# uwoseis/zephyr

Hardware: AMD Instinct MI355X
Metric: wavefields/sec (freq x source solves/s) on 1024^2 grid (higher is better)
Workload: dtype f64

## Files before the change

__graft_entry__.py:

```python
import os
import subprocess
import sys

ROOT = os.path.dirname(os.path.abspath(__file__))
CSRC = os.path.join(ROOT, 'zephyr_amd', 'csrc')
LIB = os.path.join(ROOT, 'zephyr_amd', 'libhelm.so')
SOURCES = ['assemble.hip', 'stencil.hip', 'vector.hip', 'mg.hip', 'helm3d.hip', 'mg3d.hip', 'mg3_keep.hip', 'mg3_coarse.hip', 'mg3_depth.hip', 'nd_plan.hip', 'nd_gemm.hip', 'nd_gj.hip', 'nd_leaf.hip', 'nd_factor.hip',
           'nd_passes.hip', 'nd_resid.hip', 'regrid.hip', 'runtime.hip', 'krylov.hip', 'solve_direct.hip', 'capi.hip', 'survey.hip', 'survey_frechet.hip', 'survey_hessian.hip', 'survey_newton.hip', 'survey_joint.hip',
           'survey_visco.hip', 'survey_eurus.hip']
HEADERS = ['helm_internal.hpp', 'mz_row.hpp', 'eu_row.hpp', 'solve_internal.hpp', 'mg3_internal.hpp', 'direct.hpp', 'nd_internal.hpp', 'nd_gemm_body.hpp', 'nd_gj32w.hpp', 'survey_internal.hpp']
HIPCC = os.environ.get('HIPCC', '/opt/rocm/bin/hipcc')
FLAGS = ['--offload-arch=gfx950', '-O3', '-std=c++17', '-fPIC', '-ffp-contract=fast-honor-pragmas', '-Wno-unused-value', '-Wno-unused-result']


def _stale(target, deps):
    if not os.path.exists(target):
        return True
    t = os.path.getmtime(target)
    return any(os.path.getmtime(d) > t for d in deps)


def _write_build_info(objs, ran):
    import time
    lines = ['libhelm build record (written by __graft_entry__.build())', 'hipcc: %s' % HIPCC, 'flags: %s' % ' '.join(FLAGS), '']
    lines += ['commands run by the last build that compiled something:'] + (['  ' + c.replace(ROOT + os.sep, '') for c in ran] or ['  (none: everything was up to date)'])
    lines += ['', 'artefacts:']
    for pth in objs + [LIB]:
        if os.path.exists(pth):
            st = os.stat(pth)
            lines.append('  %-40s %10d bytes  %s' % (os.path.relpath(pth, ROOT), st.st_size, time.strftime('%Y-%m-%d %H:%M:%S', time.gmtime(st.st_mtime))))
    try:
        open(os.path.join(CSRC, 'BUILD_INFO.txt'), 'w').write('\n'.join(lines) + '\n')
    except OSError:
        pass


def build(force=False):
    srcs = [os.path.join(CSRC, s) for s in SOURCES]
    hdrs = [os.path.join(CSRC, h) for h in HEADERS] + [os.path.join(ROOT, 'include', 'helm.h')]
    objs, ran, todo = [], [], []
    for s in srcs:
        o = s[:-4] + '.o'
        if force or _stale(o, [s] + hdrs):
# ... 62 lines not shown
```

include/helm.h:

```cpp
#ifndef HELM_H
#define HELM_H

#include <stddef.h>

#ifdef __cplusplus
extern "C" {
#endif

typedef struct helm_op helm_op;

enum { HELM_MINIZEPHYR = 0, HELM_EURUS = 1, HELM_3D = 2  };

enum {
    HELM_BICGSTAB = 0,
    HELM_CGNR = 1,
    HELM_AUTO = 2,
    HELM_MG = 3,
    HELM_DIRECT = 4
};

enum {
    HELM_OK = 0,
    HELM_ERR_ARG = -1,
    HELM_ERR_DEVICE = -2,
// ... 207 lines not shown
    int    nd_sparse_rhs;
    int    nd_stable;
    double nd_stable_thr;
    double nd_stable_safety;
    int    nd_fused_leaf;
    int    nd_fused_leaf_min;
    int    nd_gjstep;
    int    nd_gjstep_min;
    int    nd_overlap;
    int    nd_xcd_map;
    int    nd_plans;
    int    nd_direct_out;
    int    nd_many;
    int    nd_leaf_idle;
    int    auto_direct;
    int    auto_mg3;
    int    prof_ext;
    int    ws_slots;
    int    pf_prio;
    int    mg3_keep;
    int    mg3_keep_levels;
    int    mg3_galerkin;
    int    mg3_depth_model;
    int    mg3_bt_f32;
    int    mg3_otf;
    int    mg3_f32;
    double mg3_omega;
    int    mg3_coarse;
    int    mg3_nd_leaf;
    int    mg3_bt_twist;
    double mg3_beta;
    double sync_spin_ms;
    int    sync_sleep_us;
    int    nd_fused_sep;
    int    nd_fused_sep_min;
} helm_tuning;
int helm_get_tuning(helm_tuning *out);
int helm_set_tuning(const helm_tuning *t);

int helm_direct_plan(int nz, int nx, int leaf, int *out, int cap);
int helm_direct_plan_front(int nz, int nx, int leaf, int node, long long *cells, int cap);
int helm_debug_zgemm(int device, int M, int N, int K, const double *alpha, const double *A, const double *B,
                     const double *beta, double *C, int batch);
int helm_debug_inverse(int device, int n, double *A, int batch);
int helm_debug_zgemm_bench(int device, int M, int N, int K, int batch, int variant, int reps, double *ms_out);
#define HELM_ZG_TABLE 1
#define HELM_ZG_MASKS 2
#define HELM_ZG_TM64  4
int helm_debug_zgemm_choice(int M, int N, int K, int batch, int nf_div, int force_tile, int force_slab, int have_handle, int mode, int report[5]);
typedef struct helm_zgemm_ex {
    int device, M, N, K, batch;
    int lda, ldb, ldc;
    long long sa, sb, sc;
    double alpha[2], beta[2];
    const double *A; long long a_len;
    double *B; long long b_len;
    double *C; long long c_len;
    int force_tile, force_slab;
    int xcd_map;
    int ntc;
    int zr0, zr1, zc0, zc1, sk0, sk1;
    int tm64, c_is_b;
    const int *tabB, *tabCi, *tabCo; long long tab_len;
    int tab_stride, offB, offCi, offCo;
    int ldx; long long arena_rows;
    const double *Bx, *Bx2, *Cix;
    double *Cox, *Cox2;
    int k2, cj_out; double oscale[2];
    int *act;
    int report[5];
} helm_zgemm_ex;
int helm_debug_zgemm_ex(helm_zgemm_ex *p);
#define HELM_NM_RESID         0
#define HELM_NM_PREP          1
#define HELM_NM_PACK          2
#define HELM_NM_SCATTER_ADD   3
#define HELM_NM_RECOVER_X     4
#define HELM_NM_TRANSPOSE_OUT 5
#define HELM_NM_TRANSPOSE     6
typedef struct helm_nm_stage {
    int device, stage, nz, nx;
    long long N;
    int ncol, nblk_cap;
    const double *planes; long long planes_len;
    const double *Xin; long long xin_len; int ldin;
    double *Q; long long q_len; int ldq;
    const int *qmap;
    int store, qnorm, xin_is_u, conj;
    double *Rout; long long rout_len;
    double *Uout; long long uout_len; int ldu;
    double oscale[2];
    const unsigned char *qmask;
    long long rhs_ld, row_off;
    double *rr, *qq;
    int report[5];
} helm_nm_stage;
int helm_debug_nm_stage(helm_nm_stage *p);
int helm_debug_inverse_bench(int device, int n, const double *A, int reps, int recurse_n, double *ms_out);

int helm_mg3_axis(int n, int npml, double h, double cpml, double om_re, double om_im, int level, double *x, int *lay, double *lap,
                  int *pc, double *pw, int *n_next, int *rf, double *rw);

int helm_regrid_axis(int n_in, double h_in, int n_out, double h_out, int *start, double *taps, int cap);
typedef struct helm_regrid helm_regrid;
helm_regrid *helm_regrid_create(int device, int nz_a, int nx_a, double dz_a, double dx_a, int nz_b, int nx_b, double dz_b, double dx_b,
                                double zorig, double xorig);
void helm_regrid_destroy(helm_regrid *plan);
int helm_regrid_axis_t(int n_in, double h_in, int n_out, double h_out, int *start, double *taps, int cap);
helm_regrid *helm_regrid_create_t(int device, int nz_a, int nx_a, double dz_a, double dx_a, int nz_b, int nx_b, double dz_b, double dx_b,
                                  double zorig, double xorig);
int helm_regrid_apply_device(helm_regrid *plan, helm_op *op, int k, const void *dIn, long long in_fstride, long long in_estride, void *dOut,
                             long long out_fstride, long long out_estride, double gain_re, double gain_im, double beta, const void *dMul);
int helm_regrid_apply(helm_regrid *plan, int k, const double *in, long long in_fstride, long long in_estride, double *out, long long out_fstride,
                      long long out_estride, double gain_re, double gain_im, double beta, const double *mul);

#ifdef __cplusplus
}
#endif
#endif
```

zephyr_amd/_lib.py:

```python
import ctypes
import os
import numpy as np

_HERE = os.path.dirname(os.path.abspath(__file__))
LIB_PATH = os.path.join(_HERE, 'libhelm.so')

HELM_MINIZEPHYR, HELM_EURUS, HELM_3D = 0, 1, 2
HELM_BICGSTAB, HELM_CGNR, HELM_AUTO, HELM_MG, HELM_DIRECT = 0, 1, 2, 3, 4
HELM_RHS_NODE_MAJOR, HELM_OUT_NODE_MAJOR, HELM_NODE_MAJOR = 1, 2, 3
METHODS = {'bicgstab': HELM_BICGSTAB, 'cgnr': HELM_CGNR, 'auto': HELM_AUTO, 'mg': HELM_MG, 'direct': HELM_DIRECT}

ERRORS = {-1: 'HELM_ERR_ARG', -2: 'HELM_ERR_DEVICE', -3: 'HELM_ERR_STATE', -4: 'HELM_ERR_UNSUPPORTED', -5: 'HELM_ERR_PML'}


class HelmError(RuntimeError):
    def __init__(self, code, text):
        self.code = code
        RuntimeError.__init__(self, '%s: %s' % (ERRORS.get(code, code), text))


class SolveOpts(ctypes.Structure):
    _fields_ = [('method', ctypes.c_int), ('rtol', ctypes.c_double), ('maxit', ctypes.c_int),
                ('check_every', ctypes.c_int), ('batch', ctypes.c_int), ('flags', ctypes.c_int)]


class SolveInfo(ctypes.Structure):
    _fields_ = [('iterations', ctypes.c_int), ('status', ctypes.c_int), ('restarts', ctypes.c_int),
                ('method', ctypes.c_int), ('relres', ctypes.c_double)]


class Timing(ctypes.Structure):
    _fields_ = [('solve_ms', ctypes.c_double), ('apply_ms', ctypes.c_double),
                ('apply_launches', ctypes.c_longlong), ('apply_bytes', ctypes.c_double),
                ('factor_ms', ctypes.c_double), ('gemm_ms', ctypes.c_double),
                ('gemm_launches', ctypes.c_longlong), ('gemm_flops', ctypes.c_double),
                ('gemm_big_ms', ctypes.c_double), ('gemm_big_launches', ctypes.c_longlong), ('gemm_big_flops', ctypes.c_double),
                ('gemm_bytes', ctypes.c_double), ('gemm_sol_ms', ctypes.c_double)]


class Tuning(ctypes.Structure):
    _fields_ = [('nd_leaf', ctypes.c_int), ('nd_ws_gb', ctypes.c_double), ('nd_sparse_rhs', ctypes.c_int), ('nd_stable', ctypes.c_int),
                ('nd_stable_thr', ctypes.c_double), ('nd_stable_safety', ctypes.c_double), ('nd_fused_leaf', ctypes.c_int),
                ('nd_fused_leaf_min', ctypes.c_int), ('nd_gjstep', ctypes.c_int), ('nd_gjstep_min', ctypes.c_int), ('nd_overlap', ctypes.c_int),
                ('nd_xcd_map', ctypes.c_int), ('nd_plans', ctypes.c_int), ('nd_direct_out', ctypes.c_int), ('nd_many', ctypes.c_int), ('nd_leaf_idle', ctypes.c_int), ('auto_direct', ctypes.c_int),
                ('auto_mg3', ctypes.c_int), ('prof_ext', ctypes.c_int), ('ws_slots', ctypes.c_int), ('pf_prio', ctypes.c_int),
                ('mg3_keep', ctypes.c_int), ('mg3_keep_levels', ctypes.c_int), ('mg3_galerkin', ctypes.c_int), ('mg3_depth_model', ctypes.c_int),
                ('mg3_bt_f32', ctypes.c_int), ('mg3_otf', ctypes.c_int), ('mg3_f32', ctypes.c_int), ('mg3_omega', ctypes.c_double),
                ('mg3_coarse', ctypes.c_int), ('mg3_nd_leaf', ctypes.c_int), ('mg3_bt_twist', ctypes.c_int), ('mg3_beta', ctypes.c_double), ('sync_spin_ms', ctypes.c_double), ('sync_sleep_us', ctypes.c_int),
                ('nd_fused_sep', ctypes.c_int), ('nd_fused_sep_min', ctypes.c_int)]


class RuntimeStats(ctypes.Structure):
    _fields_ = [('dev_allocs', ctypes.c_longlong), ('dev_alloc_bytes', ctypes.c_double), ('dev_alloc_ms', ctypes.c_double),
                ('host_allocs', ctypes.c_longlong), ('host_alloc_bytes', ctypes.c_double), ('host_alloc_ms', ctypes.c_double),
                ('events_created', ctypes.c_longlong), ('streams_created', ctypes.c_longlong),
                ('first_launches', ctypes.c_longlong), ('first_launch_ms', ctypes.c_double),
                ('kernels_registered', ctypes.c_longlong), ('kernels_resolved', ctypes.c_longlong), ('warm_ms', ctypes.c_double),
                ('dev_frees', ctypes.c_longlong), ('dev_free_ms', ctypes.c_double),
                ('sync_calls', ctypes.c_longlong), ('sync_ms', ctypes.c_double), ('slow_syncs', ctypes.c_longlong), ('worst_sync_ms', ctypes.c_double)]


class ZgemmEx(ctypes.Structure):
    _fields_ = [('device', ctypes.c_int), ('M', ctypes.c_int), ('N', ctypes.c_int), ('K', ctypes.c_int), ('batch', ctypes.c_int),
                ('lda', ctypes.c_int), ('ldb', ctypes.c_int), ('ldc', ctypes.c_int),
                ('sa', ctypes.c_longlong), ('sb', ctypes.c_longlong), ('sc', ctypes.c_longlong),
                ('alpha', ctypes.c_double * 2), ('beta', ctypes.c_double * 2),
                ('A', ctypes.c_void_p), ('a_len', ctypes.c_longlong), ('B', ctypes.c_void_p), ('b_len', ctypes.c_longlong),
                ('C', ctypes.c_void_p), ('c_len', ctypes.c_longlong),
                ('force_tile', ctypes.c_int), ('force_slab', ctypes.c_int), ('xcd_map', ctypes.c_int), ('ntc', ctypes.c_int),
                ('zr0', ctypes.c_int), ('zr1', ctypes.c_int), ('zc0', ctypes.c_int), ('zc1', ctypes.c_int), ('sk0', ctypes.c_int), ('sk1', ctypes.c_int),
                ('tm64', ctypes.c_int), ('c_is_b', ctypes.c_int),
                ('tabB', ctypes.c_void_p), ('tabCi', ctypes.c_void_p), ('tabCo', ctypes.c_void_p), ('tab_len', ctypes.c_longlong),
                ('tab_stride', ctypes.c_int), ('offB', ctypes.c_int), ('offCi', ctypes.c_int), ('offCo', ctypes.c_int),
                ('ldx', ctypes.c_int), ('arena_rows', ctypes.c_longlong),
                ('Bx', ctypes.c_void_p), ('Bx2', ctypes.c_void_p), ('Cix', ctypes.c_void_p), ('Cox', ctypes.c_void_p), ('Cox2', ctypes.c_void_p),
                ('k2', ctypes.c_int), ('cj_out', ctypes.c_int), ('oscale', ctypes.c_double * 2),
                ('act', ctypes.c_void_p), ('report', ctypes.c_int * 5)]


_c_dp = ctypes.POINTER(ctypes.c_double)
_SIGNATURES = {
    'helm_device_count': (ctypes.c_int, []),
# ... 139 lines not shown
    'helm_imaging_accumulate_c64_device': (ctypes.c_int, [ctypes.c_void_p, ctypes.c_void_p, ctypes.c_void_p, ctypes.c_void_p, ctypes.c_int,
                                                          ctypes.c_void_p, ctypes.c_void_p]),
    'helm_sample_rows_c64_device': (ctypes.c_int, [ctypes.c_void_p, ctypes.c_void_p, ctypes.c_void_p, ctypes.c_int, ctypes.c_longlong, ctypes.c_void_p,
                                                   ctypes.c_void_p, ctypes.c_void_p, ctypes.c_int, ctypes.c_longlong, ctypes.c_double, ctypes.c_double,
                                                   ctypes.c_double, ctypes.c_double, ctypes.c_void_p]),
    'helm_direct_plan': (ctypes.c_int, [ctypes.c_int, ctypes.c_int, ctypes.c_int, ctypes.c_void_p, ctypes.c_int]),
    'helm_direct_plan_front': (ctypes.c_int, [ctypes.c_int, ctypes.c_int, ctypes.c_int, ctypes.c_int, ctypes.c_void_p, ctypes.c_int]),
    'helm_mg3_axis': (ctypes.c_int, [ctypes.c_int, ctypes.c_int, ctypes.c_double, ctypes.c_double, ctypes.c_double, ctypes.c_double, ctypes.c_int,
                                     ctypes.c_void_p, ctypes.c_void_p, ctypes.c_void_p, ctypes.c_void_p, ctypes.c_void_p, ctypes.c_void_p, ctypes.c_void_p,
                                     ctypes.c_void_p]),
    'helm_debug_zgemm': (ctypes.c_int, [ctypes.c_int, ctypes.c_int, ctypes.c_int, ctypes.c_int, ctypes.c_void_p, ctypes.c_void_p,
                                        ctypes.c_void_p, ctypes.c_void_p, ctypes.c_void_p, ctypes.c_int]),
    'helm_debug_zgemm_choice': (ctypes.c_int, [ctypes.c_int] * 9 + [ctypes.POINTER(ctypes.c_int)]),
    'helm_debug_zgemm_ex': (ctypes.c_int, [ctypes.POINTER(ZgemmEx)]),
    'helm_debug_nm_stage': (ctypes.c_int, [ctypes.c_void_p]),
    'helm_debug_inverse': (ctypes.c_int, [ctypes.c_int, ctypes.c_int, ctypes.c_void_p, ctypes.c_int]),
    'helm_debug_zgemm_bench': (ctypes.c_int, [ctypes.c_int, ctypes.c_int, ctypes.c_int, ctypes.c_int, ctypes.c_int, ctypes.c_int, ctypes.c_int,
                                              ctypes.POINTER(ctypes.c_double)]),
    'helm_set_rhs_support': (ctypes.c_int, [ctypes.c_void_p, ctypes.c_void_p, ctypes.c_longlong, ctypes.c_int]),
    'helm_rhs_support_from_coo': (ctypes.c_int, [ctypes.c_void_p, ctypes.c_void_p, ctypes.c_void_p, ctypes.c_longlong, ctypes.c_void_p, ctypes.c_longlong, ctypes.c_int]),
    'helm_regrid_axis': (ctypes.c_int, [ctypes.c_int, ctypes.c_double, ctypes.c_int, ctypes.c_double, ctypes.c_void_p, ctypes.c_void_p, ctypes.c_int]),
    'helm_regrid_create': (ctypes.c_void_p, [ctypes.c_int, ctypes.c_int, ctypes.c_int, ctypes.c_double, ctypes.c_double, ctypes.c_int, ctypes.c_int,
                                             ctypes.c_double, ctypes.c_double, ctypes.c_double, ctypes.c_double]),
    'helm_regrid_axis_t': (ctypes.c_int, [ctypes.c_int, ctypes.c_double, ctypes.c_int, ctypes.c_double, ctypes.c_void_p, ctypes.c_void_p, ctypes.c_int]),
    'helm_regrid_create_t': (ctypes.c_void_p, [ctypes.c_int, ctypes.c_int, ctypes.c_int, ctypes.c_double, ctypes.c_double, ctypes.c_int, ctypes.c_int,
                                               ctypes.c_double, ctypes.c_double, ctypes.c_double, ctypes.c_double]),
    'helm_regrid_destroy': (None, [ctypes.c_void_p]),
    'helm_regrid_apply_device': (ctypes.c_int, [ctypes.c_void_p, ctypes.c_void_p, ctypes.c_int, ctypes.c_void_p, ctypes.c_longlong, ctypes.c_longlong,
                                                ctypes.c_void_p, ctypes.c_longlong, ctypes.c_longlong, ctypes.c_double, ctypes.c_double, ctypes.c_double,
                                                ctypes.c_void_p]),
    'helm_regrid_apply': (ctypes.c_int, [ctypes.c_void_p, ctypes.c_int, ctypes.c_void_p, ctypes.c_longlong, ctypes.c_longlong, ctypes.c_void_p,
                                         ctypes.c_longlong, ctypes.c_longlong, ctypes.c_double, ctypes.c_double, ctypes.c_double, ctypes.c_void_p]),
    'helm_debug_inverse_bench': (ctypes.c_int, [ctypes.c_int, ctypes.c_int, ctypes.c_void_p, ctypes.c_int, ctypes.c_int, ctypes.POINTER(ctypes.c_double)]),
}

_lib = None


def exported_symbols():
    return sorted(_SIGNATURES)


def load():
    global _lib
    if _lib is None:
        if os.environ.get('HELM_NO_TORCH_PRELOAD', '0') != '1':
            try:
                import torch
            except Exception:
                pass
        if not os.path.exists(LIB_PATH):
            raise ImportError('libhelm.so not found at %s: run `python -c "import __graft_entry__ as g; g.build()"` '
                              '(hipcc --offload-arch=gfx950).  There is no CPU fallback.' % LIB_PATH)
        lib = ctypes.CDLL(LIB_PATH)
        for name, (res, args) in _SIGNATURES.items():
            fn = getattr(lib, name)
            fn.restype = res
            fn.argtypes = args
        _lib = lib
    return _lib


def tuning():
    t = Tuning()
    check(load().helm_get_tuning(ctypes.byref(t)))
    return t
# ... 133 lines not shown
```

zephyr_amd/csrc/nd_factor.hip:

```cpp
#include "nd_internal.hpp"
#include <map>
#include <mutex>
#include <cstring>

namespace {

__device__ __forceinline__ long long mf_off(long long off, long long slot, int nf, int kf) { return (long long)nf * off + (long long)kf * slot; }
__device__ __forceinline__ cplx *front_entry(const NdDev &n, cplx *arenaF, cplx *fac, int r, int c, int nf = 1, int kf = 0, int fac_private = 0) {
    const int nmax = n.smax + n.mmax;
    if (r < n.smax) {
        return fac + (fac_private ? n.finv_off : mf_off(n.finv_off, (long long)n.smax * nmax, nf, kf)) + (long long)r * nmax + c;
    }
    return arenaF + mf_off(n.foff, (long long)n.mmax * nmax, nf, kf) + (long long)(r - n.smax) * nmax + c;
}

__global__ __launch_bounds__(256) void k_nd_assemble(const NdDev *nodes, int first, cplx *arenaF, cplx *fac, const cplx *planes, int nz, int nx) {
    const NdDev n = nodes[first + blockIdx.y];
    const long long N = (long long)nz * nx;
    const int tot = n.s + n.m;
    for (int a = blockIdx.x * blockDim.x + threadIdx.x; a < n.smax; a += gridDim.x * blockDim.x)
        if (a >= n.s) *front_entry(n, arenaF, fac, a, a) = cmake(1.0, 0.0);
    for (int a = blockIdx.x * blockDim.x + threadIdx.x; a < tot; a += gridDim.x * blockDim.x) {
        int z, x, ca;
        nd_cell(n, a, z, x, ca);
// ... 269 lines not shown
                for (int q = 0; q < NK; ++q) { const int k = p + 16 * q; if (k < i) cfma(acc, rb[u][q], Bt[k][cl]); }
                load_row(rb[u], i + PD, 0, i + PD);
                #pragma unroll
                for (int off = 8; off > 0; off >>= 1) { acc.x += __shfl_xor(acc.x, off); acc.y += __shfl_xor(acc.y, off); }
                if (p == 0) Bt[i][cl] = csub(Bt[i][cl], acc);
                __builtin_amdgcn_wave_barrier();
            }
        }
    }
    #pragma unroll
    for (int u = 0; u < PD; ++u) load_row(rb[u], n - 1 - u, n - 1 - u, n);
    for (int i0 = n - 1; i0 >= 0; i0 -= PD) {
        #pragma unroll
        for (int u = 0; u < PD; ++u) {
            const int i = i0 - u;
            if (i >= 0) {
                cplx acc = cmake(0.0, 0.0), d = cmake(1.0, 0.0);
                #pragma unroll
                for (int q = 0; q < NK; ++q) { const int k = p + 16 * q; if (k > i && k < n) cfma(acc, rb[u][q], Bt[k][cl]); if (k == i) d = rb[u][q]; }
                load_row(rb[u], i - PD, i - PD, n);
                #pragma unroll
                for (int off = 8; off > 0; off >>= 1) { acc.x += __shfl_xor(acc.x, off); acc.y += __shfl_xor(acc.y, off); }
                const int src = (lane & 48) | (i & 15);
                const double dx = __shfl(d.x, src), dy = __shfl(d.y, src);
                if (p == 0) Bt[i][cl] = cmul(csub(Bt[i][cl], acc), crecip(cmake(dx, dy)));
                __builtin_amdgcn_wave_barrier();
            }
        }
    }
    __syncthreads();
    for (int e = tid; e < n * 16; e += 256) { const int i = e >> 4, c = e & 15; if (j0 + c < ncols) B[(long long)i * ldb + j0 + c] = Bt[i][c]; }
}

}

void launch_lu_solve(hipStream_t st, const cplx *LU, int ld, int n, const int *piv, cplx *B, int ldb, int ncols) {
    HELM_LAUNCH(k_lu_solve, dim3((ncols + 15) / 16), dim3(256), 0, st, LU, ld, n, piv, B, ldb, ncols);
}

static void stable_free(NdFactor *f) {
    const int dev = f->pd ? f->pd->device : 0;
    for (NdStable &st : f->stable) {
        const size_t nmax = (size_t)st.smax + st.mmax;
        helm_pool_free(dev, st.lu, (size_t)st.smax * nmax * sizeof(cplx));
        helm_pool_free(dev, st.f21, (size_t)std::max(1, st.mmax) * st.smax * sizeof(cplx));
        helm_pool_free(dev, st.piv, (size_t)st.smax * sizeof(int));
        helm_pool_free(dev, st.vs, st.vs_elems * sizeof(cplx));
    }
    f->stable.clear();
}

struct FlagSlot { int *host = nullptr; hipEvent_t ev = nullptr; int device = 0; };
namespace { std::mutex g_flag_mu; std::map<int, std::vector<FlagSlot *>> g_flag_idle; }
FlagSlot *flag_slot_acquire(int device) {
    {
        std::lock_guard<std::mutex> lk(g_flag_mu);
        std::vector<FlagSlot *> &idle = g_flag_idle[device];
        if (!idle.empty()) { FlagSlot *s = idle.back(); idle.pop_back(); return s; }
    }
    FlagSlot *s = new FlagSlot(); s->device = device;
    s->host = (int *)helm_hostpool_alloc((ND_STABLE_CAP + 1) * sizeof(int));
    if (!s->host) { delete s; return nullptr; }
    if (hipEventCreateWithFlags(&s->ev, hipEventDisableTiming) != hipSuccess) { (void)hipGetLastError(); helm_hostpool_free(s->host, (ND_STABLE_CAP + 1) * sizeof(int)); delete s; return nullptr; }
    return s;
}
void flag_slot_release(FlagSlot *s) {
    if (!s) return;
    std::lock_guard<std::mutex> lk(g_flag_mu);
    g_flag_idle[s->device].push_back(s);
}
// ... 83 lines not shown
    {
        const hipError_t es = hipEventSynchronize(slot->ev);
        memcpy(h_list, slot->host, sizeof(h_list));
        f->flag_slot = nullptr; flag_slot_release(slot);
        if (es != hipSuccess) HELM_FAIL(op, HELM_ERR_DEVICE, "direct solver: waiting for the list of ill-conditioned fronts failed: %s", hipGetErrorString(es));
    }
    const int nflag = std::max(0, std::min(h_list[0], ND_STABLE_CAP));
    if (h_list[0] > ND_STABLE_CAP) {
        std::vector<double> eh(2 * (size_t)nf * g.cnt);
        HIP_TRY(op, hipStreamSynchronize(st));
        HIP_TRY(op, hipMemcpy(eh.data(), est, eh.size() * sizeof(double), hipMemcpyDeviceToHost));
        const double thr = f->flag_thr;
        std::vector<std::pair<double, int>> cand;
        for (int j = 0; j < g.cnt; ++j) {
            const double e = eh[(size_t)j * nf + kf] * eh[(size_t)nf * g.cnt + (size_t)j * nf + kf];
            if (!(e <= thr)) cand.push_back(std::make_pair(e == e ? e : HUGE_VAL, j));
        }
        auto worse = [](const std::pair<double, int> &a, const std::pair<double, int> &b) { return a.first != b.first ? a.first > b.first : a.second < b.second; };
        const int take = std::min<int>(nflag, (int)cand.size());
        std::partial_sort(cand.begin(), cand.begin() + take, cand.end(), worse);
        for (int q = 0; q < take; ++q) h_list[1 + q] = cand[q].second;
    }
    std::sort(h_list + 1, h_list + 1 + nflag);
    if (getenv("HELM_ND_DEBUG") && atoi(getenv("HELM_ND_DEBUG")) >= 2) {
        std::vector<double> h(2 * (size_t)nf * g.cnt);
        hipStreamSynchronize(st);
        hipMemcpy(h.data(), est, h.size() * sizeof(double), hipMemcpyDeviceToHost);
        double worst = 0; int wj = 0;
        for (int j = 0; j < g.cnt; ++j) { const double e = h[(size_t)j * nf + kf] * h[(size_t)nf * g.cnt + (size_t)j * nf + kf]; if (!(e <= worst)) { worst = e; wj = j; } }
        fprintf(stderr, "[helm direct] level %d s %d cnt %d (frequency %d of %d): estimate of front 0 = %.3e * %.3e; worst %.3e at %d; flagged %d\n", g.level, g.smax, g.cnt, kf, nf, h[kf], h[(size_t)nf * g.cnt + kf], worst, wj, h_list[0]);
    }
    if ((long long)g.smax * g.mmax > P.work_elems) return HELM_OK;
    const cplx one = cmake(1, 0), mone = cmake(-1, 0);
    for (int q = 0; q < nflag; ++q) {
        const int j = h_list[1 + q];
        NdStable S;
        S.node = g.first + j; S.group = gi; S.smax = g.smax; S.mmax = g.mmax;
        S.lu = (cplx *)helm_pool_alloc(op->device, (size_t)g.smax * nmax * sizeof(cplx));
        S.f21 = (cplx *)helm_pool_alloc(op->device, (size_t)std::max(1, g.mmax) * g.smax * sizeof(cplx));
        S.piv = (int *)helm_pool_alloc(op->device, (size_t)g.smax * sizeof(int));
        f->stable.push_back(S);
        if (!S.lu || !S.f21 || !S.piv) HELM_FAIL(op, HELM_ERR_DEVICE, "direct solver: allocation for an ill-conditioned front failed");
        NdDev n = P.nodes[S.node];
        const long long foff = (long long)nf * n.foff + (long long)kf * g.mmax * nmax;
        n.finv_off = 0; n.f12_off = g.smax;
        const int rb = std::max(std::min(nmax, 4), (nmax + 2047) / 2048);
        NdPlanesSet ps; for (int q2 = 0; q2 < ND_NF_MAX; ++q2) ps.p[q2] = planes;
        HELM_LAUNCH(k_nd_build_front<true>, dim3((nmax + rb - 1) / rb, 1), dim3(256), (size_t)nmax * sizeof(int2), st, f->pd->d_nodes, 0, arenaF, S.lu, ps, P.nz, P.nx, rb,
                           0, n, nf, kf);
        cplx *F21 = arenaF + foff, *F22 = arenaF + foff + g.smax;
        HIP_TRY(op, hipMemcpy2DAsync(S.f21, (size_t)g.smax * sizeof(cplx), F21, (size_t)nmax * sizeof(cplx), (size_t)g.smax * sizeof(cplx), (size_t)g.mmax, hipMemcpyDeviceToDevice, st));
        if (g.smax <= 64) HELM_LAUNCH(k_lu_factor64, dim3(1), dim3(256), 0, st, S.lu, nmax, g.smax, S.piv);
        else HELM_LAUNCH(k_lu_factor, dim3(1), dim3(256), 0, st, S.lu, nmax, g.smax, S.piv);
        HIP_TRY(op, hipMemcpy2DAsync(work, (size_t)g.mmax * sizeof(cplx), S.lu + g.smax, (size_t)nmax * sizeof(cplx), (size_t)g.mmax * sizeof(cplx), (size_t)g.smax, hipMemcpyDeviceToDevice, st));
        HELM_LAUNCH(k_lu_solve, dim3((g.mmax + 15) / 16), dim3(256), 0, st, (const cplx *)S.lu, nmax, g.smax, (const int *)S.piv, work, g.mmax, g.mmax);
        gemm(op, g.mmax, g.mmax, g.smax, mone, S.f21, g.smax, 0, work, g.mmax, 0, one, F22, nmax, 0, 1, nullptr);
        if (getenv("HELM_ND_DEBUG") && atoi(getenv("HELM_ND_DEBUG")) >= 3) {
            auto sum2d = [&](const void *src, size_t pitch, size_t wbytes, size_t rows_) {
                std::vector<unsigned char> h(wbytes * rows_);
                hipMemcpy2D(h.data(), wbytes, src, pitch, wbytes, rows_, hipMemcpyDeviceToHost);
                unsigned long long x = 1469598103934665603ull;
                for (unsigned char c : h) { x ^= c; x *= 1099511628211ull; }
                return x;
            };
            hipStreamSynchronize(st);
            fprintf(stderr, "[helm direct] treated front %d (level %d, s %d of %d, m %d of %d): lu %016llx f12w %016llx piv %016llx f21 %016llx work %016llx f22 %016llx\n", S.node, g.level, n.s, g.smax, n.m, g.mmax,
                    sum2d(S.lu, (size_t)nmax * sizeof(cplx), (size_t)g.smax * sizeof(cplx), g.smax), sum2d(S.lu + g.smax, (size_t)nmax * sizeof(cplx), (size_t)g.mmax * sizeof(cplx), g.smax),
                    sum2d(S.piv, (size_t)g.smax * sizeof(int), (size_t)g.smax * sizeof(int), 1),
                    sum2d(S.f21, (size_t)g.smax * sizeof(cplx), (size_t)g.smax * sizeof(cplx), g.mmax), sum2d(work, (size_t)g.mmax * sizeof(cplx), (size_t)g.mmax * sizeof(cplx), g.smax),
                    sum2d(F22, (size_t)nmax * sizeof(cplx), (size_t)g.mmax * sizeof(cplx), g.mmax));
        }
    }
    const int dbg = getenv("HELM_ND_DEBUG") ? atoi(getenv("HELM_ND_DEBUG")) : 0;
    if (dbg && nflag) fprintf(stderr, "[helm direct] level %d (%s, s = %d, m = %d): %d ill-conditioned front(s) re-eliminated with a pivoted LU\n", g.level, g.leaf ? "leaves" : "separators", g.smax, g.mmax, nflag);
    return check_kernels(op, "re-elimination of ill-conditioned fronts");
}

}

int factor_group_set(helm_op *op, const FacSet &S, size_t gi, cplx *arenaF, cplx *work) {
    NdFactor *f0 = S.f[0];
    const int nf = S.nf;
    const NdPlan &P = f0->pd->plan;
    const NdDev *d_nodes = f0->pd->d_nodes;
    hipStream_t st = op->stream;
    const cplx one = cmake(1, 0), mone = cmake(-1, 0), zero = cmake(0, 0);
    const NdGroup &g = P.groups[gi];
    const int nmax = g.smax + g.mmax;
// ... 203 lines not shown
```

zephyr_amd/csrc/runtime.hip:

```cpp
#include "helm_internal.hpp"
#include <chrono>
#include <atomic>
#include <unistd.h>
#include <time.h>
#include <mutex>
#include <thread>
#include <map>
#include <cstring>
#include <algorithm>

namespace {
struct KernelRec { const void *fn; const char *pretty; std::atomic<bool> launched{false}; };
struct KernelRegistry {
    std::mutex mu;
    std::vector<KernelRec *> recs;
    std::atomic<KernelRec *> fast[2048];
    std::atomic<int> n{0};
};
KernelRegistry &kreg() { static KernelRegistry *r = new KernelRegistry(); return *r; }
struct RuntimeCounters {
    std::atomic<long long> dev_frees{0}, dev_free_us{0}, sync_calls{0}, sync_us{0}, slow_syncs{0}, worst_sync_us{0};
    std::atomic<long long> dev_allocs{0}, dev_alloc_bytes{0}, dev_alloc_us{0}, host_allocs{0}, host_alloc_bytes{0}, host_alloc_us{0},
                           events{0}, streams{0}, first_launches{0}, first_launch_us{0}, resolved{0}, warm_us{0};
};
// ... 191 lines not shown
    t.nd_sparse_rhs = helm_env_int("HELM_ND_SPARSE_RHS", 1);
    t.nd_stable = helm_env_int("HELM_ND_STABLE", 1);
    t.nd_stable_thr = tune_d("HELM_ND_STABLE_THR", 0.0);
    t.nd_stable_safety = tune_d("HELM_ND_STABLE_SAFETY", 8.0);
    t.nd_fused_leaf = helm_env_int("HELM_ND_FUSEDLEAF", 1);
    t.nd_fused_leaf_min = helm_env_int("HELM_ND_FUSEDLEAF_MIN", 2048);
    t.nd_gjstep = helm_env_int("HELM_ND_GJSTEP", 1);
    t.nd_gjstep_min = helm_env_int("HELM_ND_GJSTEP_MIN", 128);
    t.nd_overlap = helm_env_int("HELM_ND_OVERLAP_NM", 1);
    t.nd_xcd_map = helm_env_int("HELM_ND_XCDMAP", 2);
    t.nd_plans = helm_env_int("HELM_ND_PLANS", 6);
    t.nd_direct_out = helm_env_int("HELM_ND_DIRECT_OUT", 1);
    t.nd_leaf_idle = helm_env_int("HELM_ND_LEAF_IDLE", 1);
    t.nd_many = helm_env_int("HELM_ND_MANY", 1);
    t.auto_direct = helm_env_int("HELM_AUTO_DIRECT", 1);
    t.auto_mg3 = helm_env_int("HELM_AUTO_MG3", 1);
    t.prof_ext = helm_env_int("HELM_PROF_EXT", 1);
    t.ws_slots = helm_env_int("HELM_WS_SLOTS", 3);
    t.pf_prio = helm_env_int("HELM_PF_PRIO", 1);
    t.mg3_keep = helm_env_int("HELM_MG3_KEEP", 1);
    t.mg3_keep_levels = helm_env_int("HELM_MG3_KEEP_LEVELS", -1);
    t.mg3_galerkin = helm_env_int("HELM_MG3_GALERKIN", 1);
    t.mg3_depth_model = helm_env_int("HELM_MG3_DEPTH_MODEL", 1);
    t.mg3_bt_f32 = helm_env_int("HELM_MG3_BT_F32", 1);
    t.mg3_otf = helm_env_int("HELM_MG3_OTF", 1);
    t.mg3_f32 = helm_env_int("HELM_MG3_F32", 1);
    t.mg3_omega = tune_d("HELM_MG3_OMEGA", 0.9);
    { const char *cs = getenv("HELM_MG3_COARSE"); t.mg3_coarse = cs && !strcmp(cs, "nd") ? 1 : (cs && !strcmp(cs, "bt") ? 2 : 0); }
    t.mg3_nd_leaf = helm_env_int("HELM_MG3_ND_LEAF", 2);
    t.mg3_bt_twist = helm_env_int("HELM_MG3_BT_TWIST", 1);
    t.mg3_beta = tune_d("HELM_MG3_BETA", 0.0);
    t.sync_spin_ms = tune_d("HELM_SYNC_SPIN_MS", 0.0);
    t.sync_sleep_us = helm_env_int("HELM_SYNC_SLEEP_US", 0);
    t.nd_fused_sep = helm_env_int("HELM_ND_FUSEDSEP", 1);
    t.nd_fused_sep_min = helm_env_int("HELM_ND_FUSEDSEP_MIN", 512);
    tuning_clamp(t);
    return t;
}
extern char **environ;
static unsigned long long env_fingerprint() {
    unsigned long long h = 1469598103934665603ull;
    for (char **e = environ; e && *e; ++e) {
        const char *s = *e;
        if (s[0] != 'H' || s[1] != 'E' || s[2] != 'L' || s[3] != 'M' || s[4] != '_') continue;
        for (; *s; ++s) { h ^= (unsigned char)*s; h *= 1099511628211ull; }
        h ^= 0xff; h *= 1099511628211ull;
    }
    return h;
}
static bool g_tune_have = false; static unsigned long long g_tune_fp = 0; static helm_tuning g_tune_cached;
void helm_tuning_refresh() {
    std::lock_guard<std::mutex> lk(g_tune_mu);
    const unsigned long long now = env_fingerprint();
    if (!g_tune_have || now != g_tune_fp) { g_tune_cached = tuning_from_env(); g_tune_fp = now; g_tune_have = true; }
}
helm_tuning helm_tuning_now() {
    std::lock_guard<std::mutex> lk(g_tune_mu);
    if (g_tune_set) return g_tune_user;
    if (!g_tune_have) { g_tune_cached = tuning_from_env(); g_tune_fp = env_fingerprint(); g_tune_have = true; }
    return g_tune_cached;
}
extern "C" int helm_get_tuning(helm_tuning *out) { if (!out) return HELM_ERR_ARG; helm_tuning_refresh(); *out = helm_tuning_now(); return HELM_OK; }
extern "C" int helm_set_tuning(const helm_tuning *t) {
    std::lock_guard<std::mutex> lk(g_tune_mu);
    if (t) { g_tune_user = *t; tuning_clamp(g_tune_user); g_tune_set = true; } else g_tune_set = false;
    return HELM_OK;
// ... 524 lines not shown
```

Before: 16350.

## Add blocked panel LU factor and blocked triangular solve kernels for ND fronts

Adds a panel-blocked single-workgroup LU factorization that keeps a 16-column panel and U block row in shared memory, with register-tiled trailing updates. It also adds a blocked forward/back substitution that keeps the right-hand side tile in LDS and prefetches the next L/U block. Both are enabled by default through a new tuning flag and are used in the nested-dissection stable-front path and in launch_lu_solve. The intent is to cut global-memory traffic and synchronisation in small dense LU work. The cost is more LDS per block and more intricate pivot bookkeeping.

```diff
diff --git a/__graft_entry__.py b/__graft_entry__.py
--- a/__graft_entry__.py
+++ b/__graft_entry__.py
@@ -8,7 +8,7 @@
 SOURCES = ['assemble.hip', 'stencil.hip', 'vector.hip', 'mg.hip', 'helm3d.hip', 'mg3d.hip', 'mg3_keep.hip', 'mg3_coarse.hip', 'mg3_depth.hip', 'nd_plan.hip', 'nd_gemm.hip', 'nd_gj.hip', 'nd_leaf.hip', 'nd_factor.hip',
            'nd_passes.hip', 'nd_resid.hip', 'regrid.hip', 'runtime.hip', 'krylov.hip', 'solve_direct.hip', 'capi.hip', 'survey.hip', 'survey_frechet.hip', 'survey_hessian.hip', 'survey_newton.hip', 'survey_joint.hip',
            'survey_visco.hip', 'survey_eurus.hip']
-HEADERS = ['helm_internal.hpp', 'mz_row.hpp', 'eu_row.hpp', 'solve_internal.hpp', 'mg3_internal.hpp', 'direct.hpp', 'nd_internal.hpp', 'nd_gemm_body.hpp', 'nd_gj32w.hpp', 'survey_internal.hpp']
+HEADERS = ['helm_internal.hpp', 'mz_row.hpp', 'eu_row.hpp', 'solve_internal.hpp', 'mg3_internal.hpp', 'direct.hpp', 'nd_internal.hpp', 'nd_gemm_body.hpp', 'nd_gj32w.hpp', 'nd_lu_onchip.hpp', 'survey_internal.hpp']
 HIPCC = os.environ.get('HIPCC', '/opt/rocm/bin/hipcc')
 FLAGS = ['--offload-arch=gfx950', '-O3', '-std=c++17', '-fPIC', '-ffp-contract=fast-honor-pragmas', '-Wno-unused-value', '-Wno-unused-result']
 
diff --git a/include/helm.h b/include/helm.h
--- a/include/helm.h
+++ b/include/helm.h
@@ -263,6 +263,7 @@
     double mg3_beta;
     double sync_spin_ms;
     int    sync_sleep_us;
+    int    nd_lu_onchip;
     int    nd_fused_sep;
     int    nd_fused_sep_min;
 } helm_tuning;
@@ -328,6 +329,8 @@
 } helm_nm_stage;
 int helm_debug_nm_stage(helm_nm_stage *p);
 int helm_debug_inverse_bench(int device, int n, const double *A, int reps, int recurse_n, double *ms_out);
+int helm_debug_lu(int device, int n, int ld, double *A, int *piv_out, double *B, int ldb, int ncols, int onchip);
+int helm_debug_lu_bench(int device, int n, int ld, int ncols, int onchip, int reps, double *ms_factor, double *ms_solve);
 
 int helm_mg3_axis(int n, int npml, double h, double cpml, double om_re, double om_im, int level, double *x, int *lay, double *lap,
                   int *pc, double *pw, int *n_next, int *rf, double *rw);
diff --git a/zephyr_amd/_lib.py b/zephyr_amd/_lib.py
--- a/zephyr_amd/_lib.py
+++ b/zephyr_amd/_lib.py
@@ -47,7 +47,7 @@
                 ('mg3_keep', ctypes.c_int), ('mg3_keep_levels', ctypes.c_int), ('mg3_galerkin', ctypes.c_int), ('mg3_depth_model', ctypes.c_int),
                 ('mg3_bt_f32', ctypes.c_int), ('mg3_otf', ctypes.c_int), ('mg3_f32', ctypes.c_int), ('mg3_omega', ctypes.c_double),
                 ('mg3_coarse', ctypes.c_int), ('mg3_nd_leaf', ctypes.c_int), ('mg3_bt_twist', ctypes.c_int), ('mg3_beta', ctypes.c_double), ('sync_spin_ms', ctypes.c_double), ('sync_sleep_us', ctypes.c_int),
-                ('nd_fused_sep', ctypes.c_int), ('nd_fused_sep_min', ctypes.c_int)]
+                ('nd_lu_onchip', ctypes.c_int), ('nd_fused_sep', ctypes.c_int), ('nd_fused_sep_min', ctypes.c_int)]
 
 
 class RuntimeStats(ctypes.Structure):
@@ -253,6 +253,9 @@
     'helm_regrid_apply': (ctypes.c_int, [ctypes.c_void_p, ctypes.c_int, ctypes.c_void_p, ctypes.c_longlong, ctypes.c_longlong, ctypes.c_void_p,
                                          ctypes.c_longlong, ctypes.c_longlong, ctypes.c_double, ctypes.c_double, ctypes.c_double, ctypes.c_void_p]),
     'helm_debug_inverse_bench': (ctypes.c_int, [ctypes.c_int, ctypes.c_int, ctypes.c_void_p, ctypes.c_int, ctypes.c_int, ctypes.POINTER(ctypes.c_double)]),
+    'helm_debug_lu': (ctypes.c_int, [ctypes.c_int, ctypes.c_int, ctypes.c_int, ctypes.c_void_p, ctypes.c_void_p, ctypes.c_void_p, ctypes.c_int, ctypes.c_int, ctypes.c_int]),
+    'helm_debug_lu_bench': (ctypes.c_int, [ctypes.c_int, ctypes.c_int, ctypes.c_int, ctypes.c_int, ctypes.c_int, ctypes.c_int, ctypes.POINTER(ctypes.c_double),
+                                           ctypes.POINTER(ctypes.c_double)]),
 }
 
 _lib = None
diff --git a/zephyr_amd/csrc/nd_factor.hip b/zephyr_amd/csrc/nd_factor.hip
--- a/zephyr_amd/csrc/nd_factor.hip
+++ b/zephyr_amd/csrc/nd_factor.hip
@@ -325,10 +325,76 @@
     for (int e = tid; e < n * 16; e += 256) { const int i = e >> 4, c = e & 15; if (j0 + c < ncols) B[(long long)i * ldb + j0 + c] = Bt[i][c]; }
 }
 
+
+#include "nd_lu_onchip.hpp"
+
+void launch_lu_factor_sel(hipStream_t st, cplx *A, int ld, int n, int *piv, int onchip) {
+    if (onchip) HELM_LAUNCH(k_lu_factor_onchip, dim3(1), dim3(256), 0, st, A, ld, n, piv);
+    else if (n <= 64) HELM_LAUNCH(k_lu_factor64, dim3(1), dim3(256), 0, st, A, ld, n, piv);
+    else HELM_LAUNCH(k_lu_factor, dim3(1), dim3(256), 0, st, A, ld, n, piv);
+}
+void launch_lu_solve_sel(hipStream_t st, const cplx *LU, int ld, int n, const int *piv, cplx *B, int ldb, int ncols, int onchip) {
+    if (onchip) HELM_LAUNCH(k_lu_solve_blocked, dim3((ncols + 15) / 16), dim3(256), 0, st, LU, ld, n, piv, B, ldb, ncols);
+    else HELM_LAUNCH(k_lu_solve, dim3((ncols + 15) / 16), dim3(256), 0, st, LU, ld, n, piv, B, ldb, ncols);
+}
+
 }
 
 void launch_lu_solve(hipStream_t st, const cplx *LU, int ld, int n, const int *piv, cplx *B, int ldb, int ncols) {
-    HELM_LAUNCH(k_lu_solve, dim3((ncols + 15) / 16), dim3(256), 0, st, LU, ld, n, piv, B, ldb, ncols);
+    launch_lu_solve_sel(st, LU, ld, n, piv, B, ldb, ncols, helm_tuning_now().nd_lu_onchip);
+}
+
+extern "C" int helm_debug_lu(int device, int n, int ld, double *A, int *piv_out, double *B, int ldb, int ncols, int onchip) {
+    if (n < 1 || n > LUS_NMAX || ld < n || !A || !piv_out || ncols < 0 || (ncols > 0 && (!B || ldb < ncols))) return HELM_ERR_ARG;
+    helm_tuning_refresh();
+    if (hipSetDevice(device) != hipSuccess) return HELM_ERR_DEVICE;
+    cplx *dA = nullptr, *dB = nullptr; int *dP = nullptr;
+    const size_t na = (size_t)n * ld, nbb = (size_t)n * std::max(1, ldb);
+    if (hipMalloc((void **)&dA, na * 16) != hipSuccess || hipMalloc((void **)&dP, (size_t)n * sizeof(int)) != hipSuccess || (ncols > 0 && hipMalloc((void **)&dB, nbb * 16) != hipSuccess)) {
+        (void)hipGetLastError(); hipFree(dA); hipFree(dP); hipFree(dB); return HELM_ERR_DEVICE;
+    }
+    hipMemcpy(dA, A, na * 16, hipMemcpyHostToDevice);
+    if (ncols > 0) hipMemcpy(dB, B, nbb * 16, hipMemcpyHostToDevice);
+    launch_lu_factor_sel(nullptr, dA, ld, n, dP, onchip);
+    if (ncols > 0) launch_lu_solve_sel(nullptr, dA, ld, n, dP, dB, ldb, ncols, onchip);
+    const hipError_t e = hipDeviceSynchronize();
+    hipMemcpy(A, dA, na * 16, hipMemcpyDeviceToHost);
+    hipMemcpy(piv_out, dP, (size_t)n * sizeof(int), hipMemcpyDeviceToHost);
+    if (ncols > 0) hipMemcpy(B, dB, nbb * 16, hipMemcpyDeviceToHost);
+    hipFree(dA); hipFree(dP); hipFree(dB);
+    return e == hipSuccess ? HELM_OK : HELM_ERR_DEVICE;
+}
+
+extern "C" int helm_debug_lu_bench(int device, int n, int ld, int ncols, int onchip, int reps, double *ms_factor, double *ms_solve) {
+    if (n < 1 || n > LUS_NMAX || ld < n || ncols < 1 || reps < 1 || !ms_factor || !ms_solve) return HELM_ERR_ARG;
+    helm_tuning_refresh();
+    if (hipSetDevice(device) != hipSuccess) return HELM_ERR_DEVICE;
+    const size_t na = (size_t)n * ld, nbb = (size_t)n * ncols;
+    std::vector<cplx> hA(na), hB(nbb);
+    unsigned long long x = 88172645463325252ull;
+    auto rnd = [&]() { x ^= x << 13; x ^= x >> 7; x ^= x << 17; return (double)(x >> 11) / 9007199254740992.0 - 0.5; };
+    for (size_t i = 0; i < na; ++i) hA[i] = cmake(rnd(), rnd());
+    for (size_t i = 0; i < nbb; ++i) hB[i] = cmake(rnd(), rnd());
+    cplx *dA = nullptr, *dA0 = nullptr, *dB = nullptr; int *dP = nullptr;
+    if (hipMalloc((void **)&dA, na * 16) != hipSuccess || hipMalloc((void **)&dA0, na * 16) != hipSuccess || hipMalloc((void **)&dB, nbb * 16) != hipSuccess ||
+        hipMalloc((void **)&dP, (size_t)n * sizeof(int)) != hipSuccess) { (void)hipGetLastError(); hipFree(dA); hipFree(dA0); hipFree(dB); hipFree(dP); return HELM_ERR_DEVICE; }
+    hipMemcpy(dA0, hA.data(), na * 16, hipMemcpyHostToDevice);
+    hipMemcpy(dB, hB.data(), nbb * 16, hipMemcpyHostToDevice);
+    hipEvent_t e0, e1, e2; hipEventCreate(&e0); hipEventCreate(&e1); hipEventCreate(&e2);
+    auto factor = [&]() { hipMemcpyAsync(dA, dA0, na * 16, hipMemcpyDeviceToDevice, nullptr); launch_lu_factor_sel(nullptr, dA, ld, n, dP, onchip); };
+    factor();
+    launch_lu_solve_sel(nullptr, dA, ld, n, dP, dB, ncols, ncols, onchip);
+    hipEventRecord(e0, nullptr);
+    for (int r = 0; r < reps; ++r) factor();
+    hipEventRecord(e1, nullptr);
+    for (int r = 0; r < reps; ++r) launch_lu_solve_sel(nullptr, dA, ld, n, dP, dB, ncols, ncols, onchip);
+    hipEventRecord(e2, nullptr);
+    const hipError_t e = hipEventSynchronize(e2);
+    float f = 0.f, s = 0.f; hipEventElapsedTime(&f, e0, e1); hipEventElapsedTime(&s, e1, e2);
+    *ms_factor = f / reps; *ms_solve = s / reps;
+    hipEventDestroy(e0); hipEventDestroy(e1); hipEventDestroy(e2);
+    hipFree(dA); hipFree(dA0); hipFree(dB); hipFree(dP);
+    return e == hipSuccess ? HELM_OK : HELM_ERR_DEVICE;
 }
 
 static void stable_free(NdFactor *f) {
@@ -478,6 +544,7 @@
     }
     if ((long long)g.smax * g.mmax > P.work_elems) return HELM_OK;
     const cplx one = cmake(1, 0), mone = cmake(-1, 0);
+    const int lu_onchip = helm_tuning_now().nd_lu_onchip;
     for (int q = 0; q < nflag; ++q) {
         const int j = h_list[1 + q];
         NdStable S;
@@ -496,10 +563,9 @@
                            0, n, nf, kf);
         cplx *F21 = arenaF + foff, *F22 = arenaF + foff + g.smax;
         HIP_TRY(op, hipMemcpy2DAsync(S.f21, (size_t)g.smax * sizeof(cplx), F21, (size_t)nmax * sizeof(cplx), (size_t)g.smax * sizeof(cplx), (size_t)g.mmax, hipMemcpyDeviceToDevice, st));
-        if (g.smax <= 64) HELM_LAUNCH(k_lu_factor64, dim3(1), dim3(256), 0, st, S.lu, nmax, g.smax, S.piv);
-        else HELM_LAUNCH(k_lu_factor, dim3(1), dim3(256), 0, st, S.lu, nmax, g.smax, S.piv);
+        launch_lu_factor_sel(st, S.lu, nmax, g.smax, S.piv, lu_onchip);
         HIP_TRY(op, hipMemcpy2DAsync(work, (size_t)g.mmax * sizeof(cplx), S.lu + g.smax, (size_t)nmax * sizeof(cplx), (size_t)g.mmax * sizeof(cplx), (size_t)g.smax, hipMemcpyDeviceToDevice, st));
-        HELM_LAUNCH(k_lu_solve, dim3((g.mmax + 15) / 16), dim3(256), 0, st, (const cplx *)S.lu, nmax, g.smax, (const int *)S.piv, work, g.mmax, g.mmax);
+        launch_lu_solve_sel(st, S.lu, nmax, g.smax, S.piv, work, g.mmax, g.mmax, lu_onchip);
         gemm(op, g.mmax, g.mmax, g.smax, mone, S.f21, g.smax, 0, work, g.mmax, 0, one, F22, nmax, 0, 1, nullptr);
         if (getenv("HELM_ND_DEBUG") && atoi(getenv("HELM_ND_DEBUG")) >= 3) {
             auto sum2d = [&](const void *src, size_t pitch, size_t wbytes, size_t rows_) {
diff --git a/zephyr_amd/csrc/nd_lu_onchip.hpp b/zephyr_amd/csrc/nd_lu_onchip.hpp
--- /dev/null
+++ b/zephyr_amd/csrc/nd_lu_onchip.hpp
@@ -0,0 +1,223 @@
+#pragma once
+
+constexpr int LUO_PW = 16;
+constexpr int LUO_W = LUS_NMAX - LUO_PW;
+
+__device__ __forceinline__ void lu_update(cplx &a, const cplx l, const cplx u) {
+    a.x = fma(-l.x, u.x, a.x); a.x = fma(l.y, u.y, a.x);
+    a.y = fma(-l.x, u.y, a.y); a.y = fma(-l.y, u.x, a.y);
+}
+
+__global__ __launch_bounds__(256) void k_lu_factor_onchip(cplx *A, int ld, int n, int *piv) {
+    __shared__ cplx P[LUS_NMAX][LUO_PW + 1];
+    __shared__ cplx T[LUO_PW][LUO_W];
+    __shared__ double redv[2];
+    __shared__ int redi[2];
+    __shared__ int pivL[LUO_PW], tsrc[LUO_PW], ddst[LUO_PW], dsrc[LUO_PW];
+    const int tid = threadIdx.x, lane = tid & 63, wv = tid >> 6;
+    for (int p0 = 0; p0 < n; p0 += LUO_PW) {
+        const int pw = min(LUO_PW, n - p0);
+        const int w = n - pw;
+        const int w2 = n - p0 - pw;
+        for (int e = tid; e < (n - p0) * LUO_PW; e += 256) { const int i = p0 + (e >> 4), c = e & 15; if (c < pw) P[i][c] = A[(long long)i * ld + p0 + c]; }
+        __syncthreads();
+        for (int kk = 0; kk < pw; ++kk) {
+            const int k = p0 + kk;
+            double best = -1.0; int bi = k;
+            if (tid >= k && tid < n) { const double v = cabs2(P[tid][kk]); if (v > best) { best = v; bi = tid; } }
+            if (wv < 2) {
+                #pragma unroll
+                for (int o = 32; o > 0; o >>= 1) {
+                    const double v2 = __shfl_xor(best, o); const int i2 = __shfl_xor(bi, o);
+                    if (v2 > best || (v2 == best && i2 < bi)) { best = v2; bi = i2; }
+                }
+                if (lane == 0) { redv[wv] = best; redi[wv] = bi; }
+            }
+            __syncthreads();
+            int p = redi[0];
+            { const double v0 = redv[0], v1 = redv[1]; const int i1 = redi[1]; if (v1 > v0 || (v1 == v0 && i1 < p)) p = i1; }
+            if (tid == 0) { pivL[kk] = p; piv[k] = p; }
+            if (p != k && tid < pw) { const cplx t = P[k][tid]; P[k][tid] = P[p][tid]; P[p][tid] = t; }
+            __syncthreads();
+            const cplx d = crecip(P[k][kk]);
+            if (tid > k && tid < n) {
+                const cplx l = cmul(P[tid][kk], d);
+                P[tid][kk] = l;
+                for (int c = kk + 1; c < pw; ++c) { cplx a = P[tid][c]; lu_update(a, l, P[k][c]); P[tid][c] = a; }
+            }
+        }
+        __syncthreads();
+        for (int e = tid; e < (n - p0) * LUO_PW; e += 256) { const int i = p0 + (e >> 4), c = e & 15; if (c < pw) A[(long long)i * ld + p0 + c] = P[i][c]; }
+        if (tid < 2 * LUO_PW) {
+            const int s = tid & 15;
+            const bool top = tid < LUO_PW;
+            int pos = s < pw ? (top ? p0 + s : pivL[s]) : -1;
+            const int at = pos;
+            for (int kk = pw - 1; kk >= 0; --kk) { const int k = p0 + kk, p = pivL[kk]; pos = pos == k ? p : (pos == p ? k : pos); }
+            if (top) tsrc[s] = pos;
+            else { ddst[s] = at >= p0 + pw ? at : -1; dsrc[s] = pos; }
+        }
+        __syncthreads();
+        cplx dv[(LUO_PW * LUO_W + 255) / 256];
+        if (w > 0) {
+            for (int e = tid; e < pw * w; e += 256) { const int r = e / w, cj = e - r * w; T[r][cj] = A[(long long)tsrc[r] * ld + (cj < p0 ? cj : cj + pw)]; }
+            #pragma unroll
+            for (int q = 0; q < (LUO_PW * LUO_W + 255) / 256; ++q) {
+                const int e = tid + 256 * q, s = e / w, cj = e - s * w;
+                const bool ok = s < LUO_PW && ddst[s < LUO_PW ? s : 0] >= 0;
+                dv[q] = ok ? A[(long long)dsrc[s] * ld + (cj < p0 ? cj : cj + pw)] : cmake(0.0, 0.0);
+            }
+        }
+        __syncthreads();
+        if (w > 0) {
+            #pragma unroll
+            for (int q = 0; q < (LUO_PW * LUO_W + 255) / 256; ++q) {
+                const int e = tid + 256 * q, s = e / w, cj = e - s * w;
+                if (s < LUO_PW && ddst[s < LUO_PW ? s : 0] >= 0) A[(long long)ddst[s] * ld + (cj < p0 ? cj : cj + pw)] = dv[q];
+            }
+        }
+        if (tid < w2) {
+            const int cj = p0 + tid;
+            cplx u[LUO_PW];
+            #pragma unroll
+            for (int r = 0; r < LUO_PW; ++r) u[r] = T[r][cj];
+            #pragma unroll
+            for (int kq = 0; kq < LUO_PW - 1; ++kq) {
+                #pragma unroll
+                for (int r = kq + 1; r < LUO_PW; ++r) lu_update(u[r], P[p0 + r][kq], u[kq]);
+                asm volatile("" ::: "memory");
+            }
+            #pragma unroll
+            for (int r = 1; r < LUO_PW; ++r) T[r][cj] = u[r];
+        }
+        __syncthreads();
+        if (w > 0) for (int e = tid; e < pw * w; e += 256) { const int r = e / w, cj = e - r * w; A[(long long)(p0 + r) * ld + (cj < p0 ? cj : cj + pw)] = T[r][cj]; }
+        if (w2 > 0) {
+            const int i0 = p0 + LUO_PW, tot = w2 * w2;
+            for (int e0 = 0; e0 < tot; e0 += 1024) {
+                cplx a[4]; int ii[4], jj[4];
+                #pragma unroll
+                for (int u = 0; u < 4; ++u) {
+                    const int e = e0 + 256 * u + tid;
+                    const bool ok = e < tot;
+                    ii[u] = ok ? e / w2 : -1; jj[u] = ok ? e - ii[u] * w2 : 0;
+                    a[u] = ok ? A[(long long)(i0 + ii[u]) * ld + i0 + jj[u]] : cmake(0.0, 0.0);
+                }
+                #pragma unroll 2
+                for (int kq = 0; kq < LUO_PW; ++kq) {
+                    #pragma unroll
+                    for (int u = 0; u < 4; ++u) lu_update(a[u], P[i0 + (ii[u] < 0 ? 0 : ii[u])][kq], T[kq][p0 + jj[u]]);
+                }
+                #pragma unroll
+                for (int u = 0; u < 4; ++u) if (ii[u] >= 0) A[(long long)(i0 + ii[u]) * ld + i0 + jj[u]] = a[u];
+            }
+        }
+        __syncthreads();
+    }
+}
+
+__global__ __launch_bounds__(256) void k_lu_solve_blocked(const cplx *__restrict__ LU, int ld, int n, const int *__restrict__ piv, cplx *B, int ldb, int ncols) {
+    __shared__ cplx Bt[LUS_NMAX][LUO_PW + 1];
+    __shared__ cplx Lc[LUO_W][LUO_PW];
+    __shared__ int pl[LUS_NMAX], srow[LUS_NMAX];
+    constexpr int NQ = LUO_W * LUO_PW / 256;
+    const int tid = threadIdx.x, lane = tid & 63, wv = tid >> 6;
+    const int ct = wv * 4 + (lane >> 4), rt = lane & 15;
+    const int cu = tid & 15, ru = tid >> 4;
+    const int j0 = blockIdx.x * 16;
+    const int nb = (n + LUO_PW - 1) / LUO_PW;
+    for (int i = tid; i < n; i += 256) pl[i] = piv[i];
+    __syncthreads();
+    if (tid < n) {
+        int pos = tid;
+        for (int k = n - 1; k >= 0; --k) { const int p = pl[k]; pos = pos == k ? p : (pos == p ? k : pos); }
+        srow[tid] = pos;
+    }
+    __syncthreads();
+    for (int e = tid; e < nb * LUO_PW * 16; e += 256) { const int i = e >> 4, c = e & 15; Bt[i][c] = (i < n && j0 + c < ncols) ? B[(long long)srow[i] * ldb + j0 + c] : cmake(0.0, 0.0); }
+    __syncthreads();
+    cplx tri[LUO_PW], cb[NQ];
+    auto load_block = [&](cplx (&t)[LUO_PW], cplx (&c)[NQ], int J, bool lower) {
+        const int b0 = J * LUO_PW, i = b0 + rt;
+        #pragma unroll
+        for (int kq = 0; kq < LUO_PW; ++kq) t[kq] = (i < n && b0 + kq < n) ? LU[(long long)i * ld + b0 + kq] : cmake(0.0, 0.0);
+        #pragma unroll
+        for (int q = 0; q < NQ; ++q) {
+            const int ri = ru + 16 * q, r = lower ? b0 + LUO_PW + ri : ri;
+            c[q] = ((lower ? r < n : ri < b0) && b0 + cu < n) ? LU[(long long)r * ld + b0 + cu] : cmake(0.0, 0.0);
+        }
+    };
+    load_block(tri, cb, 0, true);
+    for (int J = 0; J < nb; ++J) {
+        const int b0 = J * LUO_PW;
+        cplx b = Bt[b0 + rt][ct];
+        #pragma unroll
+        for (int kq = 0; kq < LUO_PW; ++kq) {
+            if (b0 + kq < n) {
+                const cplx y = cmake(__shfl(b.x, kq, 16), __shfl(b.y, kq, 16));
+                if (rt > kq) lu_update(b, tri[kq], y);
+            }
+        }
+        Bt[b0 + rt][ct] = b;
+        #pragma unroll
+        for (int q = 0; q < NQ; ++q) Lc[ru + 16 * q][cu] = cb[q];
+        __syncthreads();
+        if (J + 1 < nb) load_block(tri, cb, J + 1, true);
+        const int nrem = n - b0 - LUO_PW;
+        if (nrem > 0) {
+            cplx yv[LUO_PW];
+            #pragma unroll
+            for (int kq = 0; kq < LUO_PW; ++kq) yv[kq] = Bt[b0 + kq][cu];
+            #pragma unroll
+            for (int q = 0; q < NQ; ++q) {
+                const int ri = ru + 16 * q;
+                if (ri < nrem) {
+                    cplx a = Bt[b0 + LUO_PW + ri][cu];
+                    #pragma unroll
+                    for (int kq = 0; kq < LUO_PW; ++kq) lu_update(a, Lc[ri][kq], yv[kq]);
+                    Bt[b0 + LUO_PW + ri][cu] = a;
+                }
+            }
+        }
+        __syncthreads();
+    }
+    load_block(tri, cb, nb - 1, false);
+    for (int J = nb - 1; J >= 0; --J) {
+        const int b0 = J * LUO_PW;
+        cplx dg = cmake(1.0, 0.0);
+        #pragma unroll
+        for (int kq = 0; kq < LUO_PW; ++kq) if (kq == rt) dg = tri[kq];
+        const cplx rd = b0 + rt < n ? crecip(dg) : cmake(1.0, 0.0);
+        cplx b = Bt[b0 + rt][ct];
+        #pragma unroll
+        for (int kq = LUO_PW - 1; kq >= 0; --kq) {
+            if (b0 + kq < n) {
+                if (rt == kq) b = cmul(b, rd);
+                const cplx x = cmake(__shfl(b.x, kq, 16), __shfl(b.y, kq, 16));
+                if (rt < kq) lu_update(b, tri[kq], x);
+            }
+        }
+        Bt[b0 + rt][ct] = b;
+        #pragma unroll
+        for (int q = 0; q < NQ; ++q) Lc[ru + 16 * q][cu] = cb[q];
+        __syncthreads();
+        if (J > 0) {
+            load_block(tri, cb, J - 1, false);
+            cplx xv[LUO_PW];
+            #pragma unroll
+            for (int kq = 0; kq < LUO_PW; ++kq) xv[kq] = Bt[b0 + kq][cu];
+            #pragma unroll
+            for (int q = 0; q < NQ; ++q) {
+                const int ri = ru + 16 * q;
+                if (ri < b0) {
+                    cplx a = Bt[ri][cu];
+                    #pragma unroll
+                    for (int kq = LUO_PW - 1; kq >= 0; --kq) if (b0 + kq < n) lu_update(a, Lc[ri][kq], xv[kq]);
+                    Bt[ri][cu] = a;
+                }
+            }
+        }
+        __syncthreads();
+    }
+    for (int e = tid; e < n * 16; e += 256) { const int i = e >> 4, c = e & 15; if (j0 + c < ncols) B[(long long)i * ldb + j0 + c] = Bt[i][c]; }
+}
diff --git a/zephyr_amd/csrc/runtime.hip b/zephyr_amd/csrc/runtime.hip
--- a/zephyr_amd/csrc/runtime.hip
+++ b/zephyr_amd/csrc/runtime.hip
@@ -247,6 +247,7 @@
     t.mg3_beta = tune_d("HELM_MG3_BETA", 0.0);
     t.sync_spin_ms = tune_d("HELM_SYNC_SPIN_MS", 0.0);
     t.sync_sleep_us = helm_env_int("HELM_SYNC_SLEEP_US", 0);
+    t.nd_lu_onchip = helm_env_int("HELM_ND_LU_ONCHIP", 1);
     t.nd_fused_sep = helm_env_int("HELM_ND_FUSEDSEP", 1);
     t.nd_fused_sep_min = helm_env_int("HELM_ND_FUSEDSEP_MIN", 512);
     tuning_clamp(t);
```

Result: slower. 14720 (-9.9%).
